# marc345/Dense2Sparse-ViT

Hardware: AMD Instinct MI355X
Metric: training images/s, DeiT-S 224 keep_ratio=0.5 (dense-to-sparse ViT train step, teacher fwd + student fwd/bwd + AdamW) (higher is better)
Workload: dtype f32; 1 GPU; DeiT-Small 224x224 patch16, 1-stage prune keep_ratio=0.5 @ block 3 (196->98 tokens), large LN predictor, kl_div mask loss, per-GPU batch 128; global_batch=128, parallelism=dp1

## Files before the change

### dense2sparse-vit_amd/csrc/attention_f32.hip

```cpp
#include "d2s_common.h"

namespace {

#ifdef D2S_ATTN_STAMPS
__device__ unsigned long long g_attn_stamps[16 * 8192];
#define ASTAMP(i) if (threadIdx.x == 0) { const int L_ = blockIdx.y * gridDim.x + blockIdx.x; if (L_ < 8192) g_attn_stamps[16 * L_ + (i)] = __builtin_amdgcn_s_memtime(); }
#define ASTAMPR(i) if (threadIdx.x == 0) { const int L_ = blockIdx.y * gridDim.x + blockIdx.x; if (L_ < 8192) g_attn_stamps[16 * L_ + (i)] = __builtin_amdgcn_s_memrealtime(); }
#else
#define ASTAMP(i)
#define ASTAMPR(i)
#endif

constexpr int DH = 64;
constexpr int PITCH = 68;

__device__ __forceinline__ void load_rows_regs(const float* __restrict__ base, long ld, int row, int nrows, int half,
                                               float scale, f32x4 (&r)[8]) {
    if (row < nrows) {
        const float* p = base + (long)row * ld + 4 * half;
#pragma unroll
        for (int t = 0; t < 8; ++t) {
            r[t] = *reinterpret_cast<const f32x4*>(p + 8 * t);
#pragma unroll
            for (int j = 0; j < 4; ++j) r[t][j] *= scale;
        }
    } else {
#pragma unroll
        for (int t = 0; t < 8; ++t) r[t] = f32x4{0.f, 0.f, 0.f, 0.f};
    }
}

__device__ __forceinline__ void tile_load(const float* __restrict__ base, long ld, int row0, int nrows, int tid, f32x4 (&r)[2]) {
#pragma unroll
    for (int i = 0; i < 2; ++i) {
        const int f = tid + i * 256, row = row0 + (f >> 4), d4 = (f & 15) * 4;
        r[i] = row < nrows ? *reinterpret_cast<const f32x4*>(base + (long)row * ld + d4) : f32x4{0.f, 0.f, 0.f, 0.f};
    }
}
__device__ __forceinline__ void tile_store(float* __restrict__ S, int tid, const f32x4 (&r)[2]) {
#pragma unroll
    for (int i = 0; i < 2; ++i) {
        const int f = tid + i * 256;
        *reinterpret_cast<f32x4*>(&S[(f >> 4) * PITCH + (f & 15) * 4]) = r[i];
    }
}

__device__ __forceinline__ void mma_lds_reg(const float* __restrict__ S, int l31, int half, const f32x4 (&y)[8], f32x16& acc) {
#pragma unroll
    for (int t = 0; t < 8; ++t) {
        const f32x4 a = *reinterpret_cast<const f32x4*>(&S[l31 * PITCH + 8 * t + 4 * half]);
#pragma unroll
        for (int j = 0; j < 4; ++j) acc = mfma32(a[j], y[t][j], acc);
    }
}
__device__ __forceinline__ void mma_reg_lds(const f32x16& p, const float* __restrict__ S, int l31, int half, f32x16 (&o)[2],
                                            int groups = 4) {
#pragma unroll
    for (int g = 0; g < 4; ++g) {
        if (g < groups) {
#pragma unroll
            for (int r = 4 * g; r < 4 * g + 4; ++r) {
                const float* row = &S[mfma32_row(r, half) * PITCH];
                o[0] = mfma32(p[r], row[l31], o[0]);
                o[1] = mfma32(p[r], row[32 + l31], o[1]);
            }
        }
    }
}

__device__ __forceinline__ void mma_lds_reg_t(const f32x16& p, const float* __restrict__ S, int l31, int half, f32x16 (&o)[2],
                                              int groups = 4) {
#pragma unroll
    for (int g = 0; g < 4; ++g) {
        if (g < groups) {
#pragma unroll
            for (int r = 4 * g; r < 4 * g + 4; ++r) {
                const float* row = &S[mfma32_row(r, half) * PITCH];
                o[0] = mfma32(row[l31], p[r], o[0]);
                o[1] = mfma32(row[32 + l31], p[r], o[1]);
            }
        }
    }
}

struct AttnFwdArgs {
    const float* qkv; float* out; float* lse; float* cls_row;
    const float* policy; float* cinv; const int* cu;
    int n, H; float scale, eps; int total;
};

template <bool POLICY, bool VARLEN>
__global__ __launch_bounds__(256, 3) void attn_fwd_kernel(AttnFwdArgs a) {
    __shared__ __attribute__((aligned(16))) float Ks[32 * PITCH];
    __shared__ __attribute__((aligned(16))) float Vs[32 * PITCH];
    __shared__ float pol_s[32];
    __shared__ __attribute__((aligned(16))) float vred[POLICY ? 16 * 64 : 4];
    __shared__ float vsum_s[64];
    extern __shared__ __attribute__((aligned(16))) float cls_s[];
    const int tid = threadIdx.x, lane = tid & 63, wave = tid >> 6, half = lane >> 5, l31 = lane & 31;
    const int H = a.H;
    ASTAMP(0); ASTAMPR(8);
    int bx, by;
    xcd_remap_2d(bx, by);
    const int b = by / H, h = by % H;
    const long ld = 3L * H * DH;
    const int row_base = VARLEN ? a.cu[b] : 0;
    const int n = VARLEN ? a.cu[b + 1] - row_base : a.n;
    if (VARLEN && bx * 128 >= n) return;
    const long tok0 = VARLEN ? (long)row_base : (long)b * n;
    const float* qb = a.qkv + tok0 * ld + h * DH;
    const float* kb = qb + (long)H * DH;
    const float* vb = kb + (long)H * DH;
    const float* polb = POLICY ? a.policy + (long)b * n : nullptr;
    const float scale = a.scale;
    const int q0 = bx * 128 + wave * 32;
    const bool active = q0 < n;
    const bool want_cls = a.cls_row != nullptr && bx == 0 && wave == 0;
    const int qi = q0 + l31;

    f32x4 qreg[8];
    load_rows_regs(qb, ld, qi, n, half, scale, qreg);

    f32x16 o[2];
#pragma unroll
    for (int r = 0; r < 16; ++r) { o[0][r] = 0.f; o[1][r] = 0.f; }
    float m_run = -INFINITY, l_run = 0.f;
    f32x4 vacc = {0.f, 0.f, 0.f, 0.f};

    const int ntiles = (n + 31) / 32;
    f32x4 kr[2], vr[2];
    float pr = 0.f;
    tile_load(kb, ld, 0, n, tid, kr);
    tile_load(vb, ld, 0, n, tid, vr);
    if (POLICY && tid < 32) pr = tid < n ? polb[tid] : 0.f;
    for (int t = 0; t < ntiles; ++t) {
        __syncthreads();
        tile_store(Ks, tid, kr);
        tile_store(Vs, tid, vr);
        if (POLICY) {
            if (tid < 32) pol_s[tid] = pr;
            vacc += vr[0];
            vacc += vr[1];
        }
        __syncthreads();
        if (t == 0) { ASTAMP(1); }
        if (t == 1) { ASTAMP(2); }
        if (t == 2) { ASTAMP(3); }
        if (t + 1 < ntiles) {
            tile_load(kb, ld, (t + 1) * 32, n, tid, kr);
            tile_load(vb, ld, (t + 1) * 32, n, tid, vr);
            if (POLICY && tid < 32) { const int kj = (t + 1) * 32 + tid; pr = kj < n ? polb[kj] : 0.f; }
        }
        if (!active) continue;
        f32x16 s;
#pragma unroll
        for (int r = 0; r < 16; ++r) s[r] = 0.f;
        mma_lds_reg(Ks, l31, half, qreg, s);
        const int kv0 = t * 32;
        float mt = -INFINITY;
#pragma unroll
        for (int r = 0; r < 16; ++r) {
            if (kv0 + mfma32_row(r, half) >= n) s[r] = -INFINITY;
            mt = fmaxf(mt, s[r]);
        }
        if (want_cls && l31 == 0) {
#pragma unroll
            for (int r = 0; r < 16; ++r) {
                const int key = kv0 + mfma32_row(r, half);
                if (key < n) cls_s[key] = s[r];
            }
        }
        mt = fmaxf(mt, __shfl_xor(mt, 32, 64));
        const float m_new = fmaxf(m_run, mt);
        const float alpha = __expf(m_run - m_new);
        float rs = 0.f;
#pragma unroll
        for (int r = 0; r < 16; ++r) {
            s[r] = __expf(s[r] - m_new);
            if (POLICY) {
                const int kr_ = mfma32_row(r, half);
                s[r] *= (kv0 + kr_ == qi) ? 1.f : pol_s[kr_];
            }
            rs += s[r];
        }
        rs += __shfl_xor(rs, 32, 64);
        l_run = l_run * alpha + rs;
        m_run = m_new;
#pragma unroll
        for (int r = 0; r < 16; ++r) {
            o[0][r] *= alpha;
            o[1][r] *= alpha;
        }
        mma_lds_reg_t(s, Vs, l31, half, o, min(4, (n - kv0 + 7) >> 3));
    }
    ASTAMP(4);
    const float c = POLICY ? a.eps / (float)n : 0.f;
    if (POLICY) {
        *reinterpret_cast<f32x4*>(&vred[(tid >> 4) * 64 + (tid & 15) * 4]) = vacc;
        __syncthreads();
        if (tid < 64) {
            float t = 0.f;
#pragma unroll
            for (int g = 0; g < 16; ++g) t += vred[g * 64 + tid];
            vsum_s[tid] = t * c;
        }
        __syncthreads();
    }
    if (!active) return;
    const float inv_l = 1.0f / (POLICY ? l_run + a.eps : l_run);
    if (qi < n) {
        float* p = a.out + (tok0 + qi) * H * DH + h * DH;
#pragma unroll
        for (int dt = 0; dt < 2; ++dt)
#pragma unroll
            for (int g = 0; g < 4; ++g) {
                f32x4 v;
#pragma unroll
                for (int j = 0; j < 4; ++j) {
                    float num = o[dt][4 * g + j];
                    if (POLICY) num += vsum_s[32 * dt + 8 * g + 4 * half + j];
                    v[j] = num * inv_l;
                }
                *reinterpret_cast<f32x4*>(p + 32 * dt + 8 * g + 4 * half) = v;
            }
    }
    const long stat0 = VARLEN ? (long)h * a.total + row_base : ((long)b * H + h) * n;
    if (half == 0 && qi < n) {
        if (a.lse) a.lse[stat0 + qi] = m_run + logf(POLICY ? l_run + a.eps : l_run);
        if (POLICY && a.cinv) a.cinv[stat0 + qi] = c * inv_l;
    }
    if (want_cls) {
        const float m0 = __shfl(m_run, 0, 64), il0 = __shfl(inv_l, 0, 64);
        float* cr = a.cls_row + stat0;
        for (int j = lane; j < n; j += 64) {
            float e = expf(cls_s[j] - m0);
            if (POLICY) e = e * (j == 0 ? 1.f : polb[j]) + c;
            cr[j] = e * il0;
        }
    }
    ASTAMP(5); ASTAMPR(9);
}

__global__ __launch_bounds__(256) void attn_delta_kernel(const float* __restrict__ out, const float* __restrict__ dout,
                                                         float* __restrict__ delta, long rows, int n, int H) {
    const int lane = threadIdx.x & 63;
    const long row = (long)blockIdx.x * 4 + (threadIdx.x >> 6);
    if (row >= rows) return;
    const long b = row / n, i = row - b * n;
    for (int h = 0; h < H; ++h) {
        const long e = row * H * DH + h * DH + lane;
        const float s = wave_sum(out[e] * dout[e]);
        if (lane == 0) delta[(b * H + h) * n + i] = s;
    }
}

template <bool POLICY>
__global__ __launch_bounds__(256, 3) void attn_bwd_dq_kernel(const float* __restrict__ qkv, const float* __restrict__ dout,
                                                          const float* __restrict__ lse, const float* __restrict__ delta,
                                                          float* __restrict__ dqkv, int n, int H, float scale,
                                                          const float* __restrict__ policy) {
    __shared__ __attribute__((aligned(16))) float Ks[32 * PITCH];
    __shared__ __attribute__((aligned(16))) float Vs[32 * PITCH];
    __shared__ float pol_s[32];
    const int tid = threadIdx.x, lane = tid & 63, wave = tid >> 6, half = lane >> 5, l31 = lane & 31;
    int bx, by;
    xcd_remap_2d(bx, by);
    const int b = by / H, h = by % H;
    const long ld = 3L * H * DH, ldo = (long)H * DH;
    const float* qb = qkv + (long)b * n * ld + h * DH;
    const float* kb = qb + (long)H * DH;
    const float* vb = kb + (long)H * DH;
    const float* dob = dout + (long)b * n * ldo + h * DH;
    const int q0 = bx * 128 + wave * 32;
    const bool active = q0 < n;

    f32x4 qreg[8], doreg[8];
    load_rows_regs(qb, ld, q0 + l31, n, half, scale, qreg);
    load_rows_regs(dob, ldo, q0 + l31, n, half, 1.0f, doreg);
    const bool qok = q0 + l31 < n;
    const float lse_i = qok ? lse[((long)b * H + h) * n + q0 + l31] : INFINITY;
    const float dl_i = qok ? delta[((long)b * H + h) * n + q0 + l31] : 0.f;

    f32x16 dq[2];
#pragma unroll
    for (int r = 0; r < 16; ++r) { dq[0][r] = 0.f; dq[1][r] = 0.f; }

    const int ntiles = (n + 31) / 32;
    f32x4 kr[2], vr[2];
    float pr = 0.f;
    const float* polb = POLICY ? policy + (long)b * n : nullptr;
    tile_load(kb, ld, 0, n, tid, kr);
    tile_load(vb, ld, 0, n, tid, vr);
    if (POLICY && tid < 32) pr = tid < n ? polb[tid] : 0.f;
    for (int t = 0; t < ntiles; ++t) {
        __syncthreads();
        tile_store(Ks, tid, kr);
        tile_store(Vs, tid, vr);
        if (POLICY && tid < 32) pol_s[tid] = pr;
        __syncthreads();
        if (t + 1 < ntiles) {
            tile_load(kb, ld, (t + 1) * 32, n, tid, kr);
            tile_load(vb, ld, (t + 1) * 32, n, tid, vr);
            if (POLICY && tid < 32) { const int kj = (t + 1) * 32 + tid; pr = kj < n ? polb[kj] : 0.f; }
        }
        if (!active) continue;
        f32x16 s, dp;
#pragma unroll
        for (int r = 0; r < 16; ++r) { s[r] = 0.f; dp[r] = 0.f; }
        mma_lds_reg(Ks, l31, half, qreg, s);
        mma_lds_reg(Vs, l31, half, doreg, dp);
        const int kv0 = t * 32;
#pragma unroll
        for (int r = 0; r < 16; ++r) {
            const int kr_ = mfma32_row(r, half);
            float p = (kv0 + kr_ < n) ? __expf(s[r] - lse_i) : 0.f;
            if (POLICY) p *= (kv0 + kr_ == q0 + l31) ? 1.f : pol_s[kr_];
            s[r] = p * (dp[r] - dl_i);
        }
        mma_reg_lds(s, Ks, l31, half, dq, min(4, (n - kv0 + 7) >> 3));
    }
    if (!active) return;
    float* dqb = dqkv + (long)b * n * ld + h * DH;
#pragma unroll
    for (int r = 0; r < 16; ++r) {
        const int qi = q0 + mfma32_row(r, half);
        if (qi < n) {
            float* p = dqb + (long)qi * ld;
            p[l31] = dq[0][r] * scale;
            p[32 + l31] = dq[1][r] * scale;
        }
    }
}

template <bool POLICY>
__global__ __launch_bounds__(256, 2) void attn_bwd_dkv_kernel(const float* __restrict__ qkv, const float* __restrict__ dout,
                                                           const float* __restrict__ lse, const float* __restrict__ delta,
                                                           float* __restrict__ dqkv, int n, int H, float scale,
                                                           const float* __restrict__ policy, const float* __restrict__ cinv) {
    __shared__ __attribute__((aligned(16))) float Qs[32 * PITCH];
    __shared__ __attribute__((aligned(16))) float Ds[32 * PITCH];
    __shared__ float lse_s[32], dl_s[32], ci_s[32];
    const int tid = threadIdx.x, lane = tid & 63, wave = tid >> 6, half = lane >> 5, l31 = lane & 31;
    int bx, by;
    xcd_remap_2d(bx, by);
    const int b = by / H, h = by % H;
    const long ld = 3L * H * DH, ldo = (long)H * DH;
    const float* qb = qkv + (long)b * n * ld + h * DH;
    const float* kb = qb + (long)H * DH;
    const float* vb = kb + (long)H * DH;
    const float* dob = dout + (long)b * n * ldo + h * DH;
    const float* lse_b = lse + ((long)b * H + h) * n;
    const float* dl_b = delta + ((long)b * H + h) * n;
    const int k0 = bx * 128 + wave * 32;
    const bool active = k0 < n;

    f32x4 kreg[8], vreg[8];
    load_rows_regs(kb, ld, k0 + l31, n, half, scale, kreg);
    load_rows_regs(vb, ld, k0 + l31, n, half, 1.0f, vreg);

    f32x16 dk[2], dv[2];
#pragma unroll
    for (int r = 0; r < 16; ++r) { dk[0][r] = 0.f; dk[1][r] = 0.f; dv[0][r] = 0.f; dv[1][r] = 0.f; }

    const int ntiles = (n + 31) / 32;
    f32x4 qr[2], dr[2];
    float lr = 0.f, dlr = 0.f, cir = 0.f;
    const float* ci_b = POLICY ? cinv + ((long)b * H + h) * n : nullptr;
    const float pol_key = (POLICY && k0 + l31 < n) ? policy[(long)b * n + k0 + l31] : 0.f;
    tile_load(qb, ld, 0, n, tid, qr);
    tile_load(dob, ldo, 0, n, tid, dr);
    if (tid < 32) { lr = tid < n ? lse_b[tid] : INFINITY; dlr = tid < n ? dl_b[tid] : 0.f; if (POLICY) cir = tid < n ? ci_b[tid] : 0.f; }
    for (int t = 0; t < ntiles; ++t) {
        __syncthreads();
        tile_store(Qs, tid, qr);
        tile_store(Ds, tid, dr);
        if (tid < 32) { lse_s[tid] = lr; dl_s[tid] = dlr; if (POLICY) ci_s[tid] = cir; }
        __syncthreads();
        if (t + 1 < ntiles) {
            tile_load(qb, ld, (t + 1) * 32, n, tid, qr);
            tile_load(dob, ldo, (t + 1) * 32, n, tid, dr);
            if (tid < 32) {
                const int qi = (t + 1) * 32 + tid;
                lr = qi < n ? lse_b[qi] : INFINITY;
                dlr = qi < n ? dl_b[qi] : 0.f;
                if (POLICY) cir = qi < n ? ci_b[qi] : 0.f;
            }
        }
        if (!active) continue;
        f32x16 s, dp;
#pragma unroll
        for (int r = 0; r < 16; ++r) { s[r] = 0.f; dp[r] = 0.f; }
        mma_lds_reg(Qs, l31, half, kreg, s);
        mma_lds_reg(Ds, l31, half, vreg, dp);
#pragma unroll
        for (int r = 0; r < 16; ++r) {
            const int qi = mfma32_row(r, half);
            float p = __expf(s[r] - lse_s[qi]);
            if (POLICY) p *= (t * 32 + qi == k0 + l31) ? 1.f : pol_key;
            s[r] = POLICY ? p + ci_s[qi] : p;
            dp[r] = p * (dp[r] - dl_s[qi]);
        }
        const int qgroups = min(4, (n - t * 32 + 7) >> 3);
        mma_reg_lds(s, Ds, l31, half, dv, qgroups);
        mma_reg_lds(dp, Qs, l31, half, dk, qgroups);
    }
    if (!active) return;
    float* dkb = dqkv + (long)b * n * ld + (long)H * DH + h * DH;
    float* dvb = dkb + (long)H * DH;
#pragma unroll
    for (int r = 0; r < 16; ++r) {
        const int ki = k0 + mfma32_row(r, half);
        if (ki < n) {
            float* pk = dkb + (long)ki * ld;
            float* pv = dvb + (long)ki * ld;
            pk[l31] = dk[0][r] * scale;
            pk[32 + l31] = dk[1][r] * scale;
            pv[l31] = dv[0][r];
            pv[32 + l31] = dv[1][r];
        }
    }
}

}

#ifdef D2S_ATTN_STAMPS
extern "C" int d2s_debug_read_attn_stamps(unsigned long long* host_out, int n_wg) {
    return hipMemcpyFromSymbol(host_out, HIP_SYMBOL(g_attn_stamps), (size_t)n_wg * 16 * sizeof(unsigned long long)) == hipSuccess ? 0 : -1;
}
#endif

extern "C" {

int d2s_attn_fwd_f32(const float* qkv, float* out, float* lse, float* cls_row, int B, int n, int H, float scale,
                     hipStream_t stream) {
    if (!qkv || !out || !lse || B <= 0 || n <= 0 || H <= 0 || n > 8192) return D2S_ERR_ARG;
    dim3 grid((n + 127) / 128, B * H), block(256);
    AttnFwdArgs a{qkv, out, lse, cls_row, nullptr, nullptr, nullptr, n, H, scale, 0.f, 0};
    hipLaunchKernelGGL((attn_fwd_kernel<false, false>), grid, block, cls_row ? (size_t)n * sizeof(float) : 0, stream, a);
    return d2s_check_launch();
}

int d2s_attn_policy_fwd_f32(const float* qkv, const float* policy, float* out, float* lse, float* cinv, float* cls_row, int B, int n,
                            int H, float scale, float eps, hipStream_t stream) {
    if (!qkv || !policy || !out || !lse || !cinv || B <= 0 || n <= 0 || H <= 0 || n > 8192) return D2S_ERR_ARG;
    dim3 grid((n + 127) / 128, B * H), block(256);
    AttnFwdArgs a{qkv, out, lse, cls_row, policy, cinv, nullptr, n, H, scale, eps, 0};
    hipLaunchKernelGGL((attn_fwd_kernel<true, false>), grid, block, cls_row ? (size_t)n * sizeof(float) : 0, stream, a);
    return d2s_check_launch();
}

int d2s_attn_varlen_fwd_f32(const float* qkv, const int* cu_seqlens, float* out, float* cls_row, int B, int total, int max_n, int H,
                            float scale, hipStream_t stream) {
    if (!qkv || !cu_seqlens || !out || B <= 0 || total <= 0 || max_n <= 0 || max_n > 8192 || H <= 0) return D2S_ERR_ARG;
    dim3 grid((max_n + 127) / 128, B * H), block(256);
    AttnFwdArgs a{qkv, out, nullptr, cls_row, nullptr, nullptr, cu_seqlens, 0, H, scale, 0.f, total};
    hipLaunchKernelGGL((attn_fwd_kernel<false, true>), grid, block, cls_row ? (size_t)max_n * sizeof(float) : 0, stream, a);
    return d2s_check_launch();
}

int d2s_attn_delta(const float* out, const float* dout, float* delta, int B, int n, int H, hipStream_t stream) {
    if (!out || !dout || !delta || B <= 0 || n <= 0 || H <= 0) return D2S_ERR_ARG;
    const long rows = (long)B * n;
    hipLaunchKernelGGL(attn_delta_kernel, dim3((unsigned)((rows + 3) / 4)), dim3(256), 0, stream, out, dout, delta, rows, n, H);
    return d2s_check_launch();
}

int d2s_attn_bwd_f32(const float* qkv, const float* out, const float* dout, const float* lse, float* dqkv, float* delta_ws, int B,
                     int n, int H, float scale, hipStream_t stream) {
    if (!qkv || !out || !dout || !lse || !dqkv || !delta_ws || B <= 0 || n <= 0 || H <= 0) return D2S_ERR_ARG;
    const long rows = (long)B * n;
    hipLaunchKernelGGL(attn_delta_kernel, dim3((unsigned)((rows + 3) / 4)), dim3(256), 0, stream, out, dout, delta_ws, rows, n, H);
    dim3 grid((n + 127) / 128, B * H), block(256);
    hipLaunchKernelGGL(attn_bwd_dq_kernel<false>, grid, block, 0, stream, qkv, dout, lse, delta_ws, dqkv, n, H, scale,
                       static_cast<const float*>(nullptr));
    hipLaunchKernelGGL(attn_bwd_dkv_kernel<false>, grid, block, 0, stream, qkv, dout, lse, delta_ws, dqkv, n, H, scale,
                       static_cast<const float*>(nullptr), static_cast<const float*>(nullptr));
    return d2s_check_launch();
}

int d2s_attn_policy_bwd_f32(const float* qkv, const float* policy, const float* out, const float* dout, const float* lse,
                            const float* cinv, float* dqkv, float* delta_ws, int B, int n, int H, float scale, hipStream_t stream) {
    if (!qkv || !policy || !out || !dout || !lse || !cinv || !dqkv || !delta_ws || B <= 0 || n <= 0 || H <= 0) return D2S_ERR_ARG;
    const long rows = (long)B * n;
    hipLaunchKernelGGL(attn_delta_kernel, dim3((unsigned)((rows + 3) / 4)), dim3(256), 0, stream, out, dout, delta_ws, rows, n, H);
    dim3 grid((n + 127) / 128, B * H), block(256);
    hipLaunchKernelGGL(attn_bwd_dq_kernel<true>, grid, block, 0, stream, qkv, dout, lse, delta_ws, dqkv, n, H, scale, policy);
    hipLaunchKernelGGL(attn_bwd_dkv_kernel<true>, grid, block, 0, stream, qkv, dout, lse, delta_ws, dqkv, n, H, scale, policy, cinv);
    return d2s_check_launch();
}

}
```

Measured before the change: 3580 images/s.

## Add fused one-pass attention backward kernel for short sequences

For sequences of up to 224 tokens, the delta, dQ and dK/dV backward kernels are replaced by a single kernel with one workgroup per (batch, head). Each wave holds one 32-row K/V tile in registers while query tiles stream through shared memory, so delta is computed inline and dQ partials are reduced across waves in LDS. This removes two launches, the delta workspace round trip and the repeated reads of Q, K and V. In exchange it uses a large amount of LDS per block and gives fewer, larger blocks, which can lower occupancy.

```diff
diff --git a/dense2sparse-vit_amd/csrc/attention_f32.hip b/dense2sparse-vit_amd/csrc/attention_f32.hip
--- a/dense2sparse-vit_amd/csrc/attention_f32.hip
+++ b/dense2sparse-vit_amd/csrc/attention_f32.hip
@@ -421,6 +421,199 @@
     }
 }
 
+constexpr int TPITCH = 36;
+
+template <int KS, int QG>
+__global__ __launch_bounds__(KS * QG * 64) void attn_bwd_onepass_kernel(const float* __restrict__ qkv, const float* __restrict__ out,
+                                                                         const float* __restrict__ dout, const float* __restrict__ lse,
+                                                                         float* __restrict__ dqkv, int n, int H, float scale) {
+    constexpr int NW = KS * QG, NT = NW * 64;
+    constexpr int NCH = (512 * QG + NT - 1) / NT;
+    __shared__ __attribute__((aligned(16))) float Ks[KS * 32 * PITCH];
+    __shared__ __attribute__((aligned(16))) float Qs[QG][32 * PITCH];
+    __shared__ __attribute__((aligned(16))) float Ds[QG][32 * PITCH];
+    __shared__ __attribute__((aligned(16))) float Xs[NW][32 * 64];
+    __shared__ float lse_s[QG][32], dl_s[QG][32];
+    const int tid = threadIdx.x, lane = tid & 63, wave = tid >> 6, half = lane >> 5, l31 = lane & 31;
+    const int ks = wave % KS, g = wave / KS;
+    const int b = blockIdx.x / H, h = blockIdx.x % H;
+    const long ld = 3L * H * DH, ldo = (long)H * DH;
+    const float* qb = qkv + (long)b * n * ld + h * DH;
+    const float* kb = qb + (long)H * DH;
+    const float* vb = kb + (long)H * DH;
+    const float* dob = dout + (long)b * n * ldo + h * DH;
+    const float* ob = out + (long)b * n * ldo + h * DH;
+    const float* lse_b = lse + ((long)b * H + h) * n;
+    float* dqb = dqkv + (long)b * n * ld + h * DH;
+    const int k0 = ks * 32;
+    const bool kactive = k0 < n;
+    const bool kok = k0 + l31 < n;
+    const int ntiles = (n + 31) / 32;
+    const int niter = (ntiles + QG - 1) / QG;
+
+    f32x4 kreg[8], vreg[8];
+    load_rows_regs(kb, ld, k0 + l31, n, half, 1.0f, kreg);
+    load_rows_regs(vb, ld, k0 + l31, n, half, 1.0f, vreg);
+#pragma unroll
+    for (int t = 0; t < 8; ++t) {
+        if (g == 0) *reinterpret_cast<f32x4*>(&Ks[(k0 + l31) * PITCH + 8 * t + 4 * half]) = kreg[t];
+#pragma unroll
+        for (int j = 0; j < 4; ++j) kreg[t][j] *= scale;
+    }
+
+    f32x16 dk[2], dv[2];
+#pragma unroll
+    for (int r = 0; r < 16; ++r) { dk[0][r] = 0.f; dk[1][r] = 0.f; dv[0][r] = 0.f; dv[1][r] = 0.f; }
+
+    f32x4 qr[NCH], dr[NCH], outr[NCH];
+    float lr = 0.f;
+    auto fetch = [&](int it) {
+#pragma unroll
+        for (int i = 0; i < NCH; ++i) {
+            const int c = tid + i * NT;
+            if (c < 512 * QG) {
+                const int row = (QG * it + (c >> 9)) * 32 + ((c & 511) >> 4), d4 = (c & 15) * 4;
+                const bool ok = row < n;
+                const f32x4 z = {0.f, 0.f, 0.f, 0.f};
+                qr[i] = ok ? *reinterpret_cast<const f32x4*>(qb + (long)row * ld + d4) : z;
+                dr[i] = ok ? *reinterpret_cast<const f32x4*>(dob + (long)row * ldo + d4) : z;
+                outr[i] = ok ? *reinterpret_cast<const f32x4*>(ob + (long)row * ldo + d4) : z;
+            }
+        }
+        if (tid < 32 * QG) {
+            const int row = (QG * it + (tid >> 5)) * 32 + (tid & 31);
+            lr = row < n ? lse_b[row] : INFINITY;
+        }
+    };
+    auto stage = [&]() {
+#pragma unroll
+        for (int i = 0; i < NCH; ++i) {
+            const int c = tid + i * NT;
+            if (c < 512 * QG) {
+                const int gq = c >> 9, row = (c & 511) >> 4;
+                *reinterpret_cast<f32x4*>(&Qs[gq][row * PITCH + (c & 15) * 4]) = qr[i];
+                *reinterpret_cast<f32x4*>(&Ds[gq][row * PITCH + (c & 15) * 4]) = dr[i];
+                f32x4 y = outr[i] * dr[i];
+#pragma unroll
+                for (int o = 8; o > 0; o >>= 1)
+#pragma unroll
+                    for (int j = 0; j < 4; ++j) y[j] += __shfl_xor(y[j], o, 64);
+                if ((c & 15) == 0) dl_s[gq][row] = (y[0] + y[2]) + (y[1] + y[3]);
+            }
+        }
+        if (tid < 32 * QG) lse_s[tid >> 5][tid & 31] = lr;
+    };
+
+    fetch(0);
+    stage();
+    __syncthreads();
+    for (int it = 0; it < niter; ++it) {
+        const int tq = QG * it + g;
+        const bool active = kactive && tq < ntiles;
+        if (it + 1 < niter) fetch(it + 1);
+        f32x16 s, dp;
+        if (active) {
+#pragma unroll
+            for (int r = 0; r < 16; ++r) { s[r] = 0.f; dp[r] = 0.f; }
+            mma_lds_reg(Qs[g], l31, half, kreg, s);
+            mma_lds_reg(Ds[g], l31, half, vreg, dp);
+#pragma unroll
+            for (int r = 0; r < 16; ++r) {
+                const int qi = mfma32_row(r, half);
+                const float p = kok ? __expf(s[r] - lse_s[g][qi]) : 0.f;
+                s[r] = p;
+                dp[r] = p * (dp[r] - dl_s[g][qi]);
+            }
+            const int qgroups = min(4, (n - tq * 32 + 7) >> 3);
+            mma_reg_lds(s, Ds[g], l31, half, dv, qgroups);
+            mma_reg_lds(dp, Qs[g], l31, half, dk, qgroups);
+        }
+        __syncthreads();
+        if (active) {
+            float* X = Xs[wave];
+#pragma unroll
+            for (int r = 0; r < 16; ++r) X[mfma32_row(r, half) * TPITCH + l31] = dp[r];
+            __builtin_amdgcn_fence(__ATOMIC_ACQ_REL, "wavefront");
+            __builtin_amdgcn_wave_barrier();
+            f32x16 dq[2];
+#pragma unroll
+            for (int r = 0; r < 16; ++r) { dq[0][r] = 0.f; dq[1][r] = 0.f; }
+            const int kgroups = min(4, (n - k0 + 7) >> 3);
+#pragma unroll
+            for (int gk = 0; gk < 4; ++gk) {
+                if (gk < kgroups) {
+                    const f32x4 a = *reinterpret_cast<const f32x4*>(&X[l31 * TPITCH + 8 * gk + 4 * half]);
+#pragma unroll
+                    for (int j = 0; j < 4; ++j) {
+                        const float* krow = &Ks[(k0 + 8 * gk + 4 * half + j) * PITCH];
+                        dq[0] = mfma32(a[j], krow[l31], dq[0]);
+                        dq[1] = mfma32(a[j], krow[32 + l31], dq[1]);
+                    }
+                }
+            }
+            __builtin_amdgcn_fence(__ATOMIC_ACQ_REL, "wavefront");
+            __builtin_amdgcn_wave_barrier();
+#pragma unroll
+            for (int r = 0; r < 16; ++r) {
+                X[mfma32_row(r, half) * 64 + l31] = dq[0][r];
+                X[mfma32_row(r, half) * 64 + 32 + l31] = dq[1][r];
+            }
+        }
+        if (it + 1 < niter) stage();
+        __syncthreads();
+#pragma unroll
+        for (int i = 0; i < NCH; ++i) {
+            const int c = tid + i * NT, gq = c >> 9, f = c & 511, qi = (QG * it + gq) * 32 + (f >> 4);
+            if (c < 512 * QG && qi < n) {
+                f32x4 acc = *reinterpret_cast<const f32x4*>(&Xs[gq * KS][4 * f]);
+                for (int w = 1; w < ntiles; ++w) acc += *reinterpret_cast<const f32x4*>(&Xs[gq * KS + w][4 * f]);
+#pragma unroll
+                for (int j = 0; j < 4; ++j) acc[j] *= scale;
+                *reinterpret_cast<f32x4*>(dqb + (long)qi * ld + (f & 15) * 4) = acc;
+            }
+        }
+    }
+    if (QG == 2) {
+        __syncthreads();
+        if (g == 1 && kactive) {
+            float* XK = Xs[wave];
+            float* XV = Xs[wave - KS];
+#pragma unroll
+            for (int r = 0; r < 16; ++r) {
+                const int o = mfma32_row(r, half) * 64 + l31;
+                XK[o] = dk[0][r]; XK[o + 32] = dk[1][r];
+                XV[o] = dv[0][r]; XV[o + 32] = dv[1][r];
+            }
+        }
+        __syncthreads();
+        if (g == 0 && kactive) {
+            const float* XK = Xs[wave + KS];
+            const float* XV = Xs[wave];
+#pragma unroll
+            for (int r = 0; r < 16; ++r) {
+                const int o = mfma32_row(r, half) * 64 + l31;
+                dk[0][r] += XK[o]; dk[1][r] += XK[o + 32];
+                dv[0][r] += XV[o]; dv[1][r] += XV[o + 32];
+            }
+        }
+    }
+    if (!kactive || g != 0) return;
+    float* dkb = dqb + (long)H * DH;
+    float* dvb = dkb + (long)H * DH;
+#pragma unroll
+    for (int r = 0; r < 16; ++r) {
+        const int ki = k0 + mfma32_row(r, half);
+        if (ki < n) {
+            float* pk = dkb + (long)ki * ld;
+            float* pv = dvb + (long)ki * ld;
+            pk[l31] = dk[0][r] * scale;
+            pk[32 + l31] = dk[1][r] * scale;
+            pv[l31] = dv[0][r];
+            pv[32 + l31] = dv[1][r];
+        }
+    }
+}
+
 }
 
 #ifdef D2S_ATTN_STAMPS
@@ -468,6 +661,16 @@
 int d2s_attn_bwd_f32(const float* qkv, const float* out, const float* dout, const float* lse, float* dqkv, float* delta_ws, int B,
                      int n, int H, float scale, hipStream_t stream) {
     if (!qkv || !out || !dout || !lse || !dqkv || !delta_ws || B <= 0 || n <= 0 || H <= 0) return D2S_ERR_ARG;
+    if (n <= 128) {
+        hipLaunchKernelGGL((attn_bwd_onepass_kernel<4, 2>), dim3((unsigned)(B * H)), dim3(512), 0, stream, qkv, out, dout, lse, dqkv, n, H,
+                           scale);
+        return d2s_check_launch();
+    }
+    if (n <= 224) {
+        hipLaunchKernelGGL((attn_bwd_onepass_kernel<7, 1>), dim3((unsigned)(B * H)), dim3(448), 0, stream, qkv, out, dout, lse, dqkv, n, H,
+                           scale);
+        return d2s_check_launch();
+    }
     const long rows = (long)B * n;
     hipLaunchKernelGGL(attn_delta_kernel, dim3((unsigned)((rows + 3) / 4)), dim3(256), 0, stream, out, dout, delta_ws, rows, n, H);
     dim3 grid((n + 127) / 128, B * H), block(256);
```

Result: no change. 3610 images/s (median of 6 runs) (+0.8%).
